# lionnus/I-ViT

Measured on AMD Instinct MI355X. Metric: images/sec DeiT-B INT8 @batch256, 1→8 MI355X; % INT8 MFMA peak, higher is better.
Workload: dtype int8; 1 GPU; DeiT-B INT8 integer-only forward, batch 256 per GPU, 224x224; global_batch=256, parallelism=dp1, launch=hip-graph replay, bitwidth=8, activation_ranges=power-of-two, operators=I-ViT (IVITIntLayerNorm, Shiftmax, ShiftGELU)

## Files before the change

### i-vit_amd/_lib.py

```python
from __future__ import annotations

import ctypes as C
import os
import subprocess

_HERE = os.path.dirname(os.path.abspath(__file__))
LIB_PATH = os.path.join(_HERE, "libivit_hip.so")
CSRC = os.path.join(_HERE, "csrc")

i64, i32, u32, f32, vp = C.c_int64, C.c_int32, C.c_uint32, C.c_float, C.c_void_p
ci = C.c_int

SIGNATURES = {
    "ivit_quantize_input_f32_i8": [vp, vp, i64, f32, vp],
    "ivit_quantize_patchify_f32_i8": [vp, vp, ci, ci, ci, ci, f32, vp],
    "ivit_gemm_i8_requant": [vp, i64, vp, i64, vp, vp, vp, vp, i64, ci, ci, ci, vp],
    "ivit_gemm_i8_requant_residual": [vp, i64, vp, i64, vp, vp, vp, vp, i64, u32, i32, u32, i32, vp, i64, ci, ci, ci, vp],
    "ivit_attention_fused_i8_ex": [vp, vp, ci, ci, ci, ci, u32, i32, f32, u32, i32, ci, vp],
    "ivit_layernorm_i8_ex": [vp, i64, ci, ci, vp, vp, vp, vp, vp, i64, ci, vp],
    "ivit_layernorm_i8_compat": [vp, i64, ci, ci, vp, vp, vp, vp, vp, vp, vp, i64, ci, vp],
    "ivit_attention_fused_i8_compat": [vp, vp, ci, ci, ci, ci, u32, i32, f32, u32, i32, vp, ci, vp],
    "ivit_attention_fused_i8_compat_band": [vp, vp, ci, ci, ci, ci, u32, i32, f32, u32, i32, vp, vp, ci, ci, vp],
    "ivit_attention_fused_i8_wide": [vp, vp, ci, ci, ci, ci, u32, i32, f32, u32, i32, vp, vp, ci, ci, ci, vp],
    "ivit_attention_fused_i8_long": [vp, vp, ci, ci, ci, ci, u32, i32, f32, u32, i32, vp, vp, ci, ci, vp],
# ... 60 lines not shown
    "ivit_ibert_gelu_build_lut": [f32, f32, f32, f32, f32, u32, i32, vp, vp],
    "ivit_ibert_softmax_build_table": [f32, f32, f32, f32, f32, f32, u32, i32, vp, vp],
    "ivit_attention_fused_i8_ibert": [vp, vp, ci, ci, ci, ci, u32, i32, u32, i32, vp, vp, ci, ci, vp],
    "ivit_attention_fused_i8_ibert_wide": [vp, vp, ci, ci, ci, ci, u32, i32, u32, i32, vp, vp, ci, ci, ci, vp],
    "ivit_attention_fused_i8_ibert_long": [vp, vp, ci, ci, ci, ci, u32, i32, u32, i32, vp, vp, ci, ci, vp],
    "ivit_ibert_layernorm_i8": [vp, i64, ci, ci, f32, vp, vp, f32, vp, vp, vp, i64, ci, vp],
    "ivit_ibert_layernorm_i16_i8": [vp, i64, ci, ci, f32, vp, vp, f32, vp, vp, vp, i64, vp],
    "ivit_ibert_layernorm_i16_i8_ex": [vp, i64, ci, ci, f32, vp, vp, f32, vp, vp, vp, i64, ci, vp],
    "ivit_ibert_gelu_f32_f32": [vp, i64, f32, f32, f32, f32, f32, vp, vp],
    "ivit_ibert_softmax_f32_f32": [vp, i64, ci, ci, f32, f32, f32, f32, f32, f32, u32, i32, ci, vp, i64, vp, vp],
    "ivit_ibert_layernorm_f32_f32": [vp, i64, ci, ci, vp, ci, vp, vp, f32, vp, i64, vp],
    "ivit_window_attention_i8": [vp, vp, i64, vp, vp, ci, ci, ci, ci, ci, ci, u32, i32, u32, i32, f32, u32, i32, vp],
    "ivit_window_attention_i8_compat": [vp, vp, i64, vp, vp, ci, ci, ci, ci, ci, ci, u32, i32, u32, i32, f32, u32, i32, vp, vp, vp],
    "ivit_window_attention_i8_band": [vp, vp, i64, vp, vp, ci, ci, ci, ci, ci, u32, i32, u32, i32, f32, u32, i32, vp, ci, ci, ci, ci, ci, ci, vp],
    "ivit_window_attention_i8_unwindow": [vp, vp, i64, vp, vp, ci, ci, ci, ci, ci, ci, u32, i32, u32, i32, f32, u32, i32, vp, vp,
                                          ci, ci, ci, ci, vp],
    "ivit_window_attention_i8_long": [vp, vp, i64, vp, vp, ci, ci, ci, ci, ci, ci, u32, i32, u32, i32, f32, u32, i32, vp, vp, vp, ci,
                                      ci, ci, ci, ci, ci, ci, vp],
    "ivit_eval_geometry": [ci, ci, ci, ci, vp],
    "ivit_resize_crop_workspace": [vp, ci, ci, vp, vp],
    "ivit_resize_crop_bicubic_u8": [vp, vp, vp, ci, ci, ci, ci, ci, vp, i64, vp, vp],
    "ivit_jpeg_probe": [vp, i64, vp],
    "ivit_jpeg_plan_image": [vp, i64, vp, i64, vp],
    "ivit_jpeg_workspace": [vp, i64, vp, vp, ci, vp, vp],
    "ivit_jpeg_decode_host": [vp, i64, vp, i64],
    "ivit_jpeg_decode_u8": [vp, vp, ci, i64, i64, i64, vp, i64, vp, vp, vp],
}


LAB_SIGNATURES = {
    "ivit_debug_force_small_gemm": [ci],
    "ivit_debug_set_gemm_flags": [ci],
    "ivit_debug_set_gemm_flags2": [ci],
    "ivit_debug_ln_wave_per_row": [ci],
    "ivit_debug_ln_ablate": [ci],
    "ivit_debug_ln_stream_cfg": [ci],
    "ivit_debug_ln_stamp_buffer": [vp],
    "ivit_gemm_i8_requant_gelu_ex": [vp, i64, vp, i64, vp, vp, vp, vp, vp, vp, i64, ci, ci, ci, ci, vp],
    "ivit_gemm_gelu_workspace_bytes": [ci, vp],
    "ivit_debug_set_stamp_buffer": [vp],
}
LAB_PATH = os.path.join(_HERE, "libivit_hip_lab.so")


class IvitError(RuntimeError):
    pass


def build(force: bool = False, verbose: bool = False) -> str:
    cmd = ["make", "-C", CSRC, "-j4"] + (["-B"] if force else []) + ([] if verbose else ["-s"])
    subprocess.check_call(cmd)
    return LIB_PATH


_lib = None
_lab = None
_use_lab = os.environ.get("IVIT_USE_LAB_LIBRARY") == "1"


def _load(path, signatures):
    if not os.path.exists(path):
        raise IvitError(f"{path} is missing: run `python -c 'import __graft_entry__ as g; g.build()'` "
                        "(there is no CPU / PyTorch fallback for the integer ViT path)")
    L = C.CDLL(path)
    L.ivit_version.restype = ci
    L.ivit_last_error_string.restype = C.c_char_p
# ... 57 lines not shown
```

### i-vit_amd/csrc/check_resources.py

```python
#!/usr/bin/env python3
import re
import sys

GUARDED = ("gemm_i8_wreg_kernel", "gemm_i8_pers_kernel", "gemm_i8_wp_kernel")
FIELDS = {"VGPRs": r"\bVGPRs: (\d+)", "AGPRs": r"AGPRs: (\d+)", "Scratch": r"ScratchSize \[bytes/lane\]: (\d+)",
          "Occupancy": r"Occupancy \[waves/SIMD\]: (\d+)", "VGPRSpill": r"VGPRs Spill: (\d+)", "SGPRSpill": r"SGPRs Spill: (\d+)",
          "LDS": r"LDS Size \[bytes/block\]: (\d+)"}


def parse(text):
    kernels, cur = {}, None
    for line in text.splitlines():
        m = re.search(r"Function Name: (\S+)", line)
        if m:
            cur = kernels.setdefault(m.group(1), {})
            continue
        if cur is None:
            continue
        for k, pat in FIELDS.items():
            m = re.search(pat, line)
            if m and k not in cur:
                cur[k] = int(m.group(1))
    return kernels


def occupancy_rules(path, what):
    kernels = parse(open(path, errors="replace").read())
    bad, seen = [], 0
    for name, r in sorted(kernels.items()):
        if what == "attention" and "attention_long_kernel" in name:
            m = re.search(r"attention_long_kernelILi(\d+)ELb([01])ELi(\d+)ELi(\d+)E", name)
            occ, need_no_scratch = int(m.group(4)) // 256, True
        elif what == "attention" and "attention_cls_kernel" in name:
            occ, need_no_scratch = 3, True
        elif what == "attention":
            m = re.search(r"attention_kernelILi(\d+)ELi(\d+)ELi(\d+)ELb([01])E", name)
            if not m:
# ... 62 lines not shown
```

### i-vit_amd/csrc/gemm.hip

```cpp
#include <type_traits>
#include "gemm_common.h"

namespace {

template <int EPI>
__global__ __launch_bounds__(NT) void gemm_i8_kernel(GemmArgs g)
{
    __shared__ __attribute__((aligned(16))) char smem[SMEM_BYTES + BN * 8];

    const int nblk = g.tiles_m * g.tiles_n;
    const int bid = blockIdx.x;
    const int q8 = nblk >> 3, r8 = nblk & 7, xcd = bid & 7;
    const int lid = (xcd < r8 ? xcd * (q8 + 1) : r8 * (q8 + 1) + (xcd - r8) * q8) + (bid >> 3);
    const int tm = lid / g.tiles_n, tn = lid - tm * g.tiles_n;
    const int m0 = tm * BM, n0 = tn * BN;

    const int tid = threadIdx.x;
    const int lane = tid & 63, wave = tid >> 6;
    const int wm = wave >> 1, wn = wave & 1;
    const int h = lane >> 5, l31 = lane & 31;
    if constexpr (EPI != EPI_I32 && EPI != EPI_RQ16 && EPI != EPI_RQ16_RES16) fill_rq_table(g, smem + SMEM_BYTES, n0, BN, tid);

    const int srow = tid >> 2, sc = tid & 3;
    const int8_t* ap[2];
// ... 887 lines not shown
                }
            }
            if (__builtin_amdgcn_ballot_w64(unc != 0) != 0) {
#pragma unroll
                for (int ii = 0; ii < 4; ++ii) {
                    const int c0 = 16 * min(i0 + ii, nsub - 1) + 4 * g4;
#pragma unroll
                    for (int r = 0; r < 4; ++r) {
                        const double tq = (double)acc[ii][r] * dyadic_mult(g.m[c0 + r], g.e[c0 + r]) + IVIT_MAGIC;
                        b[ii][r] = clamp_i32((int)(unsigned)__double_as_longlong(tq), -128, 127);
                    }
                }
            }
            unsigned D[4];
#pragma unroll
            for (int ii = 0; ii < 4; ++ii)
                D[ii] = __builtin_amdgcn_perm((unsigned)b[ii][1], (unsigned)b[ii][0], 0x0c0c0400u) |
                        __builtin_amdgcn_perm((unsigned)b[ii][3], (unsigned)b[ii][2], 0x04000c0cu);
            typedef unsigned v2u __attribute__((ext_vector_type(2)));
            const v2u ab = __builtin_amdgcn_permlane32_swap(D[0], D[2], false, false);
            const v2u cd = __builtin_amdgcn_permlane32_swap(D[1], D[3], false, false);
            const v2u ac = __builtin_amdgcn_permlane16_swap(ab.x, cd.x, false, false);
            const v2u bd = __builtin_amdgcn_permlane16_swap(ab.y, cd.y, false, false);
            const int ci = i0 + g4;
            if (ci < nsub && t < g.M) {
                const int4 v = make_int4((int)ac.x, (int)ac.y, (int)bd.x, (int)bd.y);
                if constexpr (EPI == EPI_QKV) *reinterpret_cast<int4*>(out + coff[4 * ci] + qrow_off) = v;
                else *reinterpret_cast<int4*>(out + (int64_t)t * g.ldo + 16 * ci) = v;
            }
        }
    }
}

#include "gemm_wp.h"

template <int EPI>
int launch_gemm(GemmArgs& g, const char* name, ivit_stream_t stream, int qkv_planes = 3)
{
    IVIT_REQUIRE(g.A && g.W && g.out, "%s: NULL operand", name);
    IVIT_REQUIRE(g.M > 0 && g.N > 0 && g.K > 0, "%s: empty problem M=%d N=%d K=%d", name, g.M, g.N, g.K);
    IVIT_REQUIRE(g.K % BK == 0, "%s: K=%d must be a multiple of %d", name, g.K, BK);
    IVIT_REQUIRE(g.lda >= g.K && g.ldw >= g.K && g.lda % 16 == 0 && g.ldw % 16 == 0,
                 "%s: lda=%lld ldw=%lld must be >= K and multiples of 16", name, (long long)g.lda, (long long)g.ldw);
    IVIT_REQUIRE(((uintptr_t)g.A % 16 == 0) && ((uintptr_t)g.W % 16 == 0) && ((uintptr_t)g.out % 16 == 0),
                 "%s: operands must be 16-byte aligned", name);
    if (EPI == EPI_I32 || EPI == EPI_RQ16 || EPI == EPI_RQ16_RES16) {
        IVIT_REQUIRE(g.N % 4 == 0 && g.ldo % 4 == 0 && g.ldo >= g.N, "%s: N=%d ldo=%lld must be multiples of 4", name,
                     g.N, (long long)g.ldo);
        if (EPI == EPI_RQ16 || EPI == EPI_RQ16_RES16)
            IVIT_REQUIRE(g.m && g.e && ((uintptr_t)g.m % 16 == 0) && ((uintptr_t)g.e % 16 == 0) && ((uintptr_t)g.out % 8 == 0),
                         "%s: requantiser tables missing or misaligned", name);
    } else {
        IVIT_REQUIRE(g.m && g.e, "%s: NULL requantiser table", name);
        IVIT_REQUIRE(((uintptr_t)g.bias % 16 == 0), "%s: bias must be 16-byte aligned", name);
        IVIT_REQUIRE(g.N % 16 == 0, "%s: N=%d must be a multiple of 16", name, g.N);
        IVIT_REQUIRE(((uintptr_t)g.m % 16 == 0) && ((uintptr_t)g.e % 16 == 0), "%s: m/e tables must be 16-byte aligned",
                     name);
    }
    if (EPI == EPI_RQ || EPI == EPI_RESID)
        IVIT_REQUIRE(g.ldo >= g.N && g.ldo % 16 == 0, "%s: ldo=%lld must be >= N and a multiple of 16", name,
                     (long long)g.ldo);
    if (EPI == EPI_RESID)
        IVIT_REQUIRE(g.res && g.ldr >= g.N && g.ldr % 16 == 0 && ((uintptr_t)g.res % 16 == 0),
                     "%s: residual operand missing or misaligned", name);
    if (EPI == EPI_RESID16 || EPI == EPI_RQ16_RES16)
        IVIT_REQUIRE(g.res && g.ldr >= g.N && g.ldr % 8 == 0 && ((uintptr_t)g.res % 16 == 0) && g.ldo >= g.N && g.ldo % 8 == 0,
                     "%s: 16-bit residual / output rows must be 16-byte aligned (ld multiples of 8 elements)", name);
    if (EPI == EPI_QKV) {
        IVIT_REQUIRE(g.tokens > 0 && g.heads > 0 && g.head_dim > 0 && g.head_dim % 16 == 0,
                     "%s: bad head geometry tokens=%d heads=%d head_dim=%d", name, g.tokens, g.heads, g.head_dim);
        IVIT_REQUIRE((int64_t)g.M * g.N < 2147483648ll, "%s: q/k/v output of %lld bytes exceeds the 2 GiB the 32-bit head-major offsets cover",
                     name, (long long)g.M * g.N);
        IVIT_REQUIRE(g.N == qkv_planes * g.heads * g.head_dim && g.M % g.tokens == 0,
                     "%s: N=%d != %d*heads*head_dim or M=%d %% tokens=%d != 0", name, g.N, qkv_planes, g.M, g.tokens);
    }
    g.flags = g_debug_flags & (31 | 128 | 256 | 512);
    g.flags2 = g_debug_flags2;
#if IVIT_LAB
    g.stamp = reinterpret_cast<unsigned long long*>(g_stamp_buf);
#endif
    const bool blocks = g.a_blocks || g.w_blocks;
    if constexpr (EPI == EPI_RQ || EPI == EPI_QKV) {
        if (!blocks && !g.w_frags && !g.out_blocks && !g.lut && !g.gelu_ws && g.M >= 8192 && g.K >= 32 && g.K <= SK_MAXK && g.K % 32 == 0 && g.N >= 16 &&
            g.N <= SK_MAXN && g.N % 16 == 0 && g.lda % 16 == 0 && g.ldw % 8 == 0 && ((uintptr_t)g.A % 16 == 0) && ((uintptr_t)g.W % 8 == 0) &&
            ((uintptr_t)g.out % 16 == 0) && (EPI == EPI_QKV || g.ldo % 16 == 0) && (EPI != EPI_QKV || g.head_dim % 16 == 0) && (int64_t)g.M * (EPI == EPI_QKV ? g.N : g.ldo) < 4294967296ll &&
            !g_force_small && !(IVIT_LAB && ((g_debug_flags2 & (1 << 20)) || (g_debug_flags & (31 | 128 | 256 | 512 | 1024))))) {
            const int nstrips = (g.M + 15) >> 4;
            const int grid = (nstrips + SK_WPB - 1) / SK_WPB < 512 ? (nstrips + SK_WPB - 1) / SK_WPB : 512;
            const bool any_k = IVIT_LAB && (g_debug_flags2 & (1 << 21));
            if (g.K == 128 && !any_k) hipLaunchKernelGGL((gemm_i8_skinny_kernel<EPI, 4>), dim3(grid), dim3(SK_NT), 0, ivit_stream(stream), g);
            else if (g.K == 64 && !any_k) hipLaunchKernelGGL((gemm_i8_skinny_kernel<EPI, 2>), dim3(grid), dim3(SK_NT), 0, ivit_stream(stream), g);
            else hipLaunchKernelGGL((gemm_i8_skinny_kernel<EPI, 0>), dim3(grid), dim3(SK_NT), 0, ivit_stream(stream), g);
            IVIT_CHECK_LAUNCH(name);
        }
    }
    if (blocks && !g.w_frags) {
        IVIT_REQUIRE(EPI != EPI_I32 && EPI != EPI_RQ16 && g.M >= 2048 && g.N >= BCH && !g_force_small,
                     "%s: block-layout operands need the persistent kernel (M >= 2048, N >= 128, requantising epilogue)", name);
        IVIT_REQUIRE(!g.a_blocks || g.lda == g.K, "%s: a block-layout A operand is dense (lda == K)", name);
        IVIT_REQUIRE(!g.w_blocks || g.ldw == g.K, "%s: a block-layout W operand is dense (ldw == K)", name);
    }
    if (g.w_frags) IVIT_REQUIRE(!g.a_blocks || g.lda == g.K, "%s: a block-layout A operand is dense (lda == K)", name);
    IVIT_REQUIRE(!g.lut || (g.w_frags && EPI == EPI_RQ), "%s: the output map needs the fragment-packed weight form (IVIT_W_FRAGS)", name);
    if (g.w_frags) {
        IVIT_REQUIRE(EPI != EPI_I32 && EPI != EPI_RQ16 && g.M >= 2048 && g.N >= 128 && g.N % 64 == 0 && (g.K / BK) % 3 == 0 && !g.w_blocks && !g_force_small,
                     "%s: the fragment-packed weight needs M >= 2048, N >= 128, N %% 64 == 0, K %% 192 == 0 and a requantising epilogue", name);
        if constexpr (EPI != EPI_I32 && EPI != EPI_RQ16) {
            g.tiles_m = (g.M + WR_TOK - 1) / WR_TOK;
            g.tiles_n = (g.N + WR_CH - 1) / WR_CH;
            g.narrow = 0;
            if constexpr (EPI == EPI_RQ || EPI == EPI_RESID || EPI == EPI_QKV) {
                if (IVIT_LAB && g.w_frags == 2 && !g.lut && !g.gelu_ws && (g_debug_flags2 & 8192) && !(g_debug_flags2 & (256 | 512))) {
                    g.narrow = 1;
                    g.tiles_n = (g.N + WR_CH / 2 - 1) / (WR_CH / 2);
                }
            }
            const int ntiles = g.tiles_m * g.tiles_n;
            if constexpr (IVIT_LAB != 0 && (EPI == EPI_RQ || EPI == EPI_QKV)) {
                if (g.w_frags == 2 && !g.lut && !g.gelu_ws && !g.narrow && (g.K / BK) >= 12 && (g_debug_flags2 & 32768) && !(g_debug_flags2 & (256 | 512)) &&
                    !(g_debug_flags & 127)) {
                    IVIT_REQUIRE(((int64_t)g.M + 16) * (EPI == EPI_QKV ? g.N : g.ldo) < 4294967296ll,
                                 "%s: IVIT_W_FRAGS16 addresses its output with 32-bit offsets: operand of 4 GiB or more", name);
                    g.split_from = ntiles;
                    if constexpr (EPI == EPI_QKV) {
                        IVIT_REQUIRE((int64_t)g.M * g.tokens < 4294967296ll, "%s: M * tokens must stay below 2^32", name);
// ... 385 lines not shown
```

### i-vit_amd/csrc/gemm_common.h

```cpp
#pragma once
#include <type_traits>

#include "common.h"

#if IVIT_LAB
extern int g_kernel_choice;
extern bool g_force_small;
extern void* g_stamp_buf;
extern int g_debug_flags;
extern int g_debug_flags2;
#else
constexpr int g_kernel_choice = 0;
constexpr bool g_force_small = false;
constexpr int g_debug_flags = 0;
constexpr int g_debug_flags2 = 0;
#endif
#ifndef IVIT_STORE_POLICY
#define IVIT_STORE_POLICY 0
#endif

namespace {

constexpr int BM = 128;
constexpr int BN = 128;
constexpr int BK = 64;
constexpr int NT = 256;
constexpr int STAGE_BYTES = (BM + BN) * BK;
constexpr int W_OFF = BM * BK;
constexpr int SMEM_BYTES = 2 * STAGE_BYTES;

enum { EPI_RQ = 0, EPI_RESID = 1, EPI_QKV = 2, EPI_I32 = 3, EPI_RESID16 = 4, EPI_RQ16 = 5, EPI_RQ16_RES16 = 6 };


struct GemmArgs {
    const int8_t* A;
    int64_t lda;
    const int8_t* W;
    int64_t ldw;
    const int32_t* bias;
    const uint32_t* m;
    const int32_t* e;
    void* out;
    int64_t ldo;
// ... 934 lines not shown
```

### i-vit_amd/csrc/gemm_lab.hip

```cpp
#include "gemm_common.h"

int g_kernel_choice = 0;
bool g_force_small = false;
void* g_stamp_buf = nullptr;
int g_debug_flags = 0;
int g_debug_flags2 = 0;

namespace {

template <int EPI, int ABL>
__global__ __launch_bounds__(BIG_NT, 2) void gemm_i8_big_kernel(GemmArgs g)
{
    __shared__ __attribute__((aligned(16))) char smem[BIG_SMEM + BCH * 8];
    unsigned long long t_start = 0, t_loop = 0, t_epi = 0, r_start = 0;
    if constexpr (ABL & 512) {
        t_start = __builtin_amdgcn_s_memtime();
        r_start = __builtin_amdgcn_s_memrealtime();
    }

    const int nblk = g.tiles_m * g.tiles_n;
    const int bid = blockIdx.x;
    const int q8 = nblk >> 3, r8 = nblk & 7, xcd = bid & 7;
    const int lid = (xcd < r8 ? xcd * (q8 + 1) : r8 * (q8 + 1) + (xcd - r8) * q8) + (bid >> 3);
    const int tm = lid / g.tiles_n, tn = lid - tm * g.tiles_n;
    const int m0 = tm * BTOK, n0 = tn * BCH;

    const int tid = threadIdx.x;
    const int lane = tid & 63, wave = __builtin_amdgcn_readfirstlane(tid >> 6);
    const int wc = wave >> 1, wt = wave & 1;
    const int h = lane >> 5, l31 = lane & 31;

    const int8_t* asrc[4];
    const int8_t* wsrc[2];
    const int lrow = lane >> 2, lslot = lane & 3;
#pragma unroll
    for (int i = 0; i < 4; ++i) {
        int row = 16 * (wave + 4 * i) + lrow;
        int c = lslot ^ ((row >> 2) & 3);
        asrc[i] = g.A + (int64_t)min(m0 + row, g.M - 1) * g.lda + 16 * c;
// ... 189 lines not shown

int ivit_gemm_lab_launch(int epi, void* gemm_args, const char* name, ivit_stream_t stream, int* rc)
{
    GemmArgs& g = *static_cast<GemmArgs*>(gemm_args);
    int handled = 0;
    switch (epi) {
        case EPI_RQ: *rc = launch_lab<EPI_RQ>(g, name, stream, &handled); break;
        case EPI_RESID: *rc = launch_lab<EPI_RESID>(g, name, stream, &handled); break;
        case EPI_QKV: *rc = launch_lab<EPI_QKV>(g, name, stream, &handled); break;
        default: break;
    }
    return handled;
}

IVIT_EXPORT int ivit_debug_force_small_gemm(int on)
{
    g_force_small = (on == 1);
    g_kernel_choice = (on == 2);
    return IVIT_OK;
}

IVIT_EXPORT int ivit_debug_set_gemm_flags(int flags)
{
    g_debug_flags = flags;
    return IVIT_OK;
}

IVIT_EXPORT int ivit_debug_set_gemm_flags2(int flags)
{
    g_debug_flags2 = flags;
    return IVIT_OK;
}

IVIT_EXPORT int ivit_debug_set_stamp_buffer(void* buf)
{
    g_stamp_buf = buf;
    return IVIT_OK;
}
```

### i-vit_amd/csrc/rowops.hip

```cpp
#include <limits.h>

#include "common.h"
#include "rowsum.h"

#if IVIT_LAB
int g_ln_wave_per_row = 0;
int g_ln_ablate = 0;
int g_ln_stream_cfg = 0;
unsigned long long* g_ln_stamps = nullptr;
#else
constexpr int g_ln_wave_per_row = 0;
constexpr int g_ln_ablate = 0;
constexpr int g_ln_stream_cfg = 0;
#endif

namespace {

typedef float v2f __attribute__((ext_vector_type(2)));

constexpr int NT = 256;
constexpr int WPB = NT / 64;

IVIT_DEV int sx8(int v, int byte) { return (int)(int8_t)(v >> (8 * byte)); }

// ... 1023 lines not shown
    if (total < 2147483648ll) {
        const unsigned w4 = (unsigned)(hw >> 2), tot = (unsigned)total;
        for (unsigned q = blockIdx.x * NT + threadIdx.x; q < tot; q += gridDim.x * NT) {
            const unsigned r = q / w4, x4 = q - r * w4;
            const unsigned r2 = r / (unsigned)hw, y = r - r2 * (unsigned)hw;
            const unsigned b = r2 / (unsigned)chans, c = r2 - b * (unsigned)chans;
            const float4 v = *reinterpret_cast<const float4*>(img + (size_t)r * hw + 4 * x4);
            const unsigned px = x4 / (unsigned)pw4, kw = (x4 - px * pw4) * 4;
            const unsigned py = y / (unsigned)patch, kh = y - py * patch;
            const int64_t row = ((int64_t)b * g + py) * g + px;
            const unsigned col = (c * patch + kh) * patch + kw;
            *reinterpret_cast<int*>(A + row * lda + col) = pack4(quant_sym_i8(v.x, inv_scale), quant_sym_i8(v.y, inv_scale),
                                                                 quant_sym_i8(v.z, inv_scale), quant_sym_i8(v.w, inv_scale));
        }
        return;
    }
    for (int64_t q = (int64_t)blockIdx.x * NT + threadIdx.x; q < total; q += (int64_t)gridDim.x * NT) {
        int x4 = (int)(q % (hw >> 2));
        int64_t r = q / (hw >> 2);
        int y = (int)(r % hw);
        r /= hw;
        int c = (int)(r % chans);
        int b = (int)(r / chans);
        float4 v = *reinterpret_cast<const float4*>(img + (((int64_t)b * chans + c) * hw + y) * hw + 4 * x4);
        int px = x4 / pw4, kw = (x4 - px * pw4) * 4;
        int py = y / patch, kh = y - py * patch;
        int64_t row = ((int64_t)b * g + py) * g + px;
        int col = (c * patch + kh) * patch + kw;
        *reinterpret_cast<int*>(A + row * lda + col) = pack4(quant_sym_i8(v.x, inv_scale), quant_sym_i8(v.y, inv_scale),
                                                             quant_sym_i8(v.z, inv_scale), quant_sym_i8(v.w, inv_scale));
    }
}

__global__ __launch_bounds__(NT) void patchify_u8_kernel(const uint8_t* img, int8_t* A, int64_t lda, int batch, int chans, int hw,
                                                         int patch, const int8_t* lut)
{
    __shared__ int8_t s_lut[4 * 256];
    for (int i = threadIdx.x; i < chans * 256; i += NT) s_lut[i] = lut[i];
    __syncthreads();
    const int g = hw / patch;
    const int pw4 = patch >> 2;
    const int64_t total = (int64_t)batch * chans * hw * (hw >> 2);
    for (int64_t q = (int64_t)blockIdx.x * NT + threadIdx.x; q < total; q += (int64_t)gridDim.x * NT) {
        int x4 = (int)(q % (hw >> 2));
        int64_t r = q / (hw >> 2);
        int y = (int)(r % hw);
        r /= hw;
        int c = (int)(r % chans);
        int b = (int)(r / chans);
        const unsigned v = *reinterpret_cast<const unsigned*>(img + (((int64_t)b * chans + c) * hw + y) * hw + 4 * x4);
        const int8_t* t = s_lut + 256 * c;
        int px = x4 / pw4, kw = (x4 - px * pw4) * 4;
        int py = y / patch, kh = y - py * patch;
        int64_t row = ((int64_t)b * g + py) * g + px;
        int col = (c * patch + kh) * patch + kw;
        *reinterpret_cast<int*>(A + row * lda + col) = pack4(t[v & 255], t[(v >> 8) & 255], t[(v >> 16) & 255], t[v >> 24]);
    }
}

__global__ __launch_bounds__(NT) void embed_kernel(const int8_t* patch, const int16_t* pos_add, const int8_t* cls_row,
                                                   double Mq, int8_t* out, int batch, int tokens, int C)
{
    const int cd = C >> 2;
    const int64_t total = (int64_t)batch * tokens * cd;
    for (int64_t q = (int64_t)blockIdx.x * NT + threadIdx.x; q < total; q += (int64_t)gridDim.x * NT) {
        int d = (int)(q % cd);
        int64_t r = q / cd;
        int tok = (int)(r % tokens);
        int b = (int)(r / tokens);
        int res;
        if (tok == 0) {
            res = *reinterpret_cast<const int*>(cls_row + 4 * d);
        } else {
            int w = *reinterpret_cast<const int*>(patch + ((int64_t)b * (tokens - 1) + tok - 1) * C + 4 * d);
            const int16_t* pa = pos_add + (int64_t)tok * C + 4 * d;
            int o[4];
#pragma unroll
            for (int c = 0; c < 4; ++c) o[c] = clamp_i32(requant_exact(sx8(w, c), Mq) + (int)pa[c], -128, 127);
            res = pack4(o[0], o[1], o[2], o[3]);
        }
        *reinterpret_cast<int*>(out + ((int64_t)b * tokens + tok) * C + 4 * d) = res;
    }
}

__global__ __launch_bounds__(NT) void embed16_kernel(const int16_t* patch, const int32_t* pos_add, const int16_t* cls_row,
                                                     double Mq, int16_t* out, int batch, int tokens, int C)
{
    const int cd = C >> 2;
    const int64_t total = (int64_t)batch * tokens * cd;
    for (int64_t q = (int64_t)blockIdx.x * NT + threadIdx.x; q < total; q += (int64_t)gridDim.x * NT) {
        const int d = (int)(q % cd);
        const int64_t r = q / cd;
        const int tok = (int)(r % tokens);
        const int b = (int)(r / tokens);
        int2 res;
        if (tok == 0) {
            res = *reinterpret_cast<const int2*>(cls_row + 4 * d);
        } else {
            const int2 w = *reinterpret_cast<const int2*>(patch + ((int64_t)b * (tokens - 1) + tok - 1) * C + 4 * d);
            const int4 pa = *reinterpret_cast<const int4*>(pos_add + (int64_t)tok * C + 4 * d);
            const int k[4] = {(int)(int16_t)w.x, w.x >> 16, (int)(int16_t)w.y, w.y >> 16};
            const int p4[4] = {pa.x, pa.y, pa.z, pa.w};
            int o[4];
#pragma unroll
            for (int c = 0; c < 4; ++c) o[c] = clamp_i32(requant_exact(k[c], Mq) + p4[c], -32768, 32767);
            res.x = (o[0] & 0xffff) | (o[1] << 16);
            res.y = (o[2] & 0xffff) | (o[3] << 16);
        }
        *reinterpret_cast<int2*>(out + ((int64_t)b * tokens + tok) * C + 4 * d) = res;
    }
}

__global__ __launch_bounds__(NT) void head_argmax_kernel(const int32_t* acc, const float* s_acc, int batch, int N,
                                                         float* logits, int32_t* top1)
// ... 641 lines not shown
    hipLaunchKernelGGL(minmax_kernel, dim3(ew_grid(n) < 2048 ? ew_grid(n) : 2048), dim3(NT), 0, st, x, n, keys);
    hipLaunchKernelGGL(minmax_finish_kernel, dim3(1), dim3(1), 0, st, keys);
    IVIT_CHECK_LAUNCH("ivit_minmax_f32");
}

IVIT_EXPORT int ivit_quantize_input_f32_i8(const float* x, int8_t* out, int64_t n, float inv_scale,
                                           ivit_stream_t stream)
{
    IVIT_REQUIRE(x && out && n > 0, "ivit_quantize_input_f32_i8: bad operand");
    IVIT_REQUIRE(((uintptr_t)x % 16 == 0) && ((uintptr_t)out % 4 == 0), "ivit_quantize_input_f32_i8: misaligned");
    hipLaunchKernelGGL(quantize_kernel, dim3(ew_grid(n / 4 + 1)), dim3(NT), 0, ivit_stream(stream), x, out, n,
                       inv_scale);
    IVIT_CHECK_LAUNCH("ivit_quantize_input_f32_i8");
}

IVIT_EXPORT int ivit_quantize_input_f32_i32(const float* x, int32_t* out, int64_t n, float inv_scale, int bits,
                                            ivit_stream_t stream)
{
    IVIT_REQUIRE(x && out && n > 0 && bits >= 2 && bits <= 32, "ivit_quantize_input_f32_i32: bad operand");
    const float lo = -__builtin_ldexpf(1.0f, bits - 1), hi = __builtin_ldexpf(1.0f, bits - 1) - 1.0f;
    hipLaunchKernelGGL(quantize_i32_kernel, dim3(ew_grid(n)), dim3(NT), 0, ivit_stream(stream), x, out, n, inv_scale, lo, hi);
    IVIT_CHECK_LAUNCH("ivit_quantize_input_f32_i32");
}

static int launch_patchify(const char* who, const float* img, int8_t* A, int64_t lda, int batch, int chans, int hw, int patch,
                           float inv_scale, ivit_stream_t stream)
{
    IVIT_REQUIRE(img && A && batch > 0 && chans > 0, "%s: bad operand", who);
    IVIT_REQUIRE(patch > 0 && patch % 4 == 0 && hw % patch == 0, "%s: hw=%d patch=%d", who, hw, patch);
    IVIT_REQUIRE(lda >= (int64_t)chans * patch * patch && lda % 4 == 0, "%s: lda=%lld too small or not a multiple of 4", who,
                 (long long)lda);
    IVIT_REQUIRE(((uintptr_t)img % 16 == 0) && ((uintptr_t)A % 4 == 0), "%s: misaligned", who);
    const int64_t total = (int64_t)batch * chans * hw * (hw / 4);
    hipLaunchKernelGGL(patchify_kernel, dim3(ew_grid(total)), dim3(NT), 0, ivit_stream(stream), img, A, lda, batch, chans,
                       hw, patch, inv_scale);
    IVIT_CHECK_LAUNCH(who);
}

IVIT_EXPORT int ivit_quantize_patchify_f32_i8(const float* img, int8_t* A, int batch, int chans, int hw, int patch,
                                              float inv_scale, ivit_stream_t stream)
{
    return launch_patchify("ivit_quantize_patchify_f32_i8", img, A, (int64_t)chans * patch * patch, batch, chans, hw, patch,
                           inv_scale, stream);
}

IVIT_EXPORT int ivit_quantize_patchify_u8_i8(const uint8_t* img, int8_t* A, int64_t lda, int batch, int chans, int hw, int patch,
                                             const int8_t* lut, ivit_stream_t stream)
{
    IVIT_REQUIRE(img && A && lut && batch > 0 && chans > 0 && chans <= 4 && hw > 0 && patch > 0 && hw % patch == 0 && patch % 4 == 0,
                 "ivit_quantize_patchify_u8_i8: bad shape (up to 4 channels, hw %% patch == 0, patch %% 4 == 0)");
    IVIT_REQUIRE(lda >= (int64_t)chans * patch * patch && lda % 4 == 0 && ((uintptr_t)img % 4 == 0) && ((uintptr_t)A % 4 == 0),
                 "ivit_quantize_patchify_u8_i8: lda too small or misaligned operand");
    const int64_t total = (int64_t)batch * chans * hw * (hw / 4);
    hipLaunchKernelGGL(patchify_u8_kernel, dim3(ew_grid(total)), dim3(NT), 0, ivit_stream(stream), img, A, lda, batch, chans, hw,
                       patch, lut);
    IVIT_CHECK_LAUNCH("ivit_quantize_patchify_u8_i8");
}

IVIT_EXPORT int ivit_quantize_patchify_ld_f32_i8(const float* img, int8_t* A, int64_t lda, int batch, int chans, int hw,
                                                 int patch, float inv_scale, ivit_stream_t stream)
{
    return launch_patchify("ivit_quantize_patchify_ld_f32_i8", img, A, lda, batch, chans, hw, patch, inv_scale, stream);
}

IVIT_EXPORT int ivit_embed_assemble_i8(const int8_t* patch, const int16_t* pos_add, const int8_t* cls_row, uint32_t m,
                                       int32_t e, int8_t* out, int batch, int tokens, int C, ivit_stream_t stream)
{
    IVIT_REQUIRE(patch && pos_add && cls_row && out, "ivit_embed_assemble_i8: NULL operand");
    IVIT_REQUIRE(batch > 0 && tokens > 1 && C > 0 && C % 4 == 0, "ivit_embed_assemble_i8: bad shape");
    IVIT_REQUIRE(((uintptr_t)patch % 4 == 0) && ((uintptr_t)out % 4 == 0) && ((uintptr_t)cls_row % 4 == 0) &&
                     ((uintptr_t)pos_add % 8 == 0),
                 "ivit_embed_assemble_i8: misaligned");
    const double Mq = ivit_dyadic_to_double(m, e);
    IVIT_REQUIRE(Mq < 1048576.0, "ivit_embed_assemble_i8: requant multiplier too large");
    const int64_t total = (int64_t)batch * tokens * (C / 4);
    hipLaunchKernelGGL(embed_kernel, dim3(ew_grid(total)), dim3(NT), 0, ivit_stream(stream), patch, pos_add, cls_row,
                       Mq, out, batch, tokens, C);
    IVIT_CHECK_LAUNCH("ivit_embed_assemble_i8");
}

IVIT_EXPORT int ivit_embed_assemble_i16(const int16_t* patch, const int32_t* pos_add, const int16_t* cls_row, uint32_t m,
                                        int32_t e, int16_t* out, int batch, int tokens, int C, ivit_stream_t stream)
{
    IVIT_REQUIRE(patch && pos_add && cls_row && out, "ivit_embed_assemble_i16: NULL operand");
    IVIT_REQUIRE(batch > 0 && tokens > 1 && C > 0 && C % 4 == 0, "ivit_embed_assemble_i16: bad shape");
    IVIT_REQUIRE(((uintptr_t)patch % 8 == 0) && ((uintptr_t)out % 8 == 0) && ((uintptr_t)cls_row % 8 == 0) &&
                     ((uintptr_t)pos_add % 16 == 0),
                 "ivit_embed_assemble_i16: misaligned");
    const double Mq = ivit_dyadic_to_double(m, e);
    IVIT_REQUIRE(Mq < 32768.0, "ivit_embed_assemble_i16: requant multiplier too large");
    const int64_t total = (int64_t)batch * tokens * (C / 4);
    hipLaunchKernelGGL(embed16_kernel, dim3(ew_grid(total)), dim3(NT), 0, ivit_stream(stream), patch, pos_add, cls_row,
                       Mq, out, batch, tokens, C);
    IVIT_CHECK_LAUNCH("ivit_embed_assemble_i16");
}

IVIT_EXPORT int ivit_head_argmax(const int32_t* acc, const float* s_acc, int batch, int N, float* logits_f32,
                                 int32_t* top1, ivit_stream_t stream)
{
    IVIT_REQUIRE(acc && s_acc && top1 && batch > 0 && N > 0, "ivit_head_argmax: bad operand");
    hipLaunchKernelGGL(head_argmax_kernel, dim3(grid_for_rows(batch)), dim3(NT), 0, ivit_stream(stream), acc, s_acc,
                       batch, N, logits_f32, top1);
    IVIT_CHECK_LAUNCH("ivit_head_argmax");
}

namespace {
template <bool F32>
void launch_head_topk(int k, const int32_t* acc, const float* s_acc, const float* logits_in, int batch, int ld, int N,
// ... 126 lines not shown
```

### include/ivit_hip_debug.h

```cpp
#ifndef IVIT_HIP_DEBUG_H
#define IVIT_HIP_DEBUG_H

#ifdef __cplusplus
extern "C" {
#endif

int ivit_debug_force_small_gemm(int on);
int ivit_debug_set_gemm_flags(int flags);
int ivit_debug_set_gemm_flags2(int flags);
int ivit_debug_set_stamp_buffer(void* buf);

int ivit_debug_ln_wave_per_row(int on);

int ivit_debug_ln_stream_cfg(int cfg);
int ivit_debug_ln_stamp_buffer(void* buf);

int ivit_debug_ln_ablate(int bits);

int ivit_gemm_gelu_workspace_bytes(int M, int64_t* bytes);
int ivit_gemm_i8_requant_gelu_ex(const int8_t* A, int64_t lda, const int8_t* W, int64_t ldw, const int32_t* bias,
                                 const uint32_t* m, const int32_t* e, const int8_t* gelu_lut, void* workspace,
                                 int8_t* out, int64_t ldo, int M, int N, int K, int layouts, ivit_stream_t stream);

#ifdef __cplusplus
}
#endif
#endif
```

Before: 42160 images/s.

## Add split-K small-M GEMM kernel and vectorized patchify/embed streaming kernels

Adds a small-M int8 GEMM kernel that tiles output as 64x32 and splits the K loop across four waves. Each wave keeps a register-prefetched pipeline of MFMA operands, then partial sums are reduced through LDS before a requant, residual or int32 epilogue. It is selected for small M/N tile counts, such as the classifier head, where the existing kernels leave most of the GPU idle. Patchify and embed-assemble also get 16-byte-per-thread streaming kernels when alignment allows. These add code paths and a debug launch counter, with some risk in the new dispatch conditions and edge handling.

Result: no change. 42560 images/s, median of 6 (+0.9%).

```diff
diff --git a/i-vit_amd/_lib.py b/i-vit_amd/_lib.py
--- a/i-vit_amd/_lib.py
+++ b/i-vit_amd/_lib.py
@@ -116,6 +116,7 @@
     "ivit_debug_force_small_gemm": [ci],
     "ivit_debug_set_gemm_flags": [ci],
     "ivit_debug_set_gemm_flags2": [ci],
+    "ivit_debug_small_m_gemm_launches": [vp],
     "ivit_debug_ln_wave_per_row": [ci],
     "ivit_debug_ln_ablate": [ci],
     "ivit_debug_ln_stream_cfg": [ci],
diff --git a/i-vit_amd/csrc/check_resources.py b/i-vit_amd/csrc/check_resources.py
--- a/i-vit_amd/csrc/check_resources.py
+++ b/i-vit_amd/csrc/check_resources.py
@@ -2,7 +2,8 @@
 import re
 import sys
 
-GUARDED = ("gemm_i8_wreg_kernel", "gemm_i8_pers_kernel", "gemm_i8_wp_kernel")
+GUARDED = ("gemm_i8_wreg_kernel", "gemm_i8_pers_kernel", "gemm_i8_wp_kernel",
+           "gemm_i8_smallm_kernel")
 FIELDS = {"VGPRs": r"\bVGPRs: (\d+)", "AGPRs": r"AGPRs: (\d+)", "Scratch": r"ScratchSize \[bytes/lane\]: (\d+)",
           "Occupancy": r"Occupancy \[waves/SIMD\]: (\d+)", "VGPRSpill": r"VGPRs Spill: (\d+)", "SGPRSpill": r"SGPRs Spill: (\d+)",
           "LDS": r"LDS Size \[bytes/block\]: (\d+)"}
diff --git a/i-vit_amd/csrc/gemm.hip b/i-vit_amd/csrc/gemm.hip
--- a/i-vit_amd/csrc/gemm.hip
+++ b/i-vit_amd/csrc/gemm.hip
@@ -943,6 +943,151 @@
     }
 }
 
+constexpr int SM_ROWS = 64, SM_CH = 32, SM_NT = 256, SM_DEPTH = 4;
+constexpr int SM_MAX_M = 1024, SM_MAX_ITEMS = 384;
+constexpr int SM_RS = SM_CH + 4;
+constexpr int SM_SMEM = 4 * SM_ROWS * SM_RS * 4;
+
+template <int EPI>
+__global__ __launch_bounds__(SM_NT) void gemm_i8_smallm_kernel(GemmArgs g)
+{
+    static_assert(EPI == EPI_RQ || EPI == EPI_RESID || EPI == EPI_I32, "small-M form: plain int8, residual and raw int32 epilogues");
+    __shared__ __attribute__((aligned(16))) int part[4 * SM_ROWS * SM_RS];
+    const int tid = threadIdx.x, lane = tid & 63, wave = tid >> 6;
+    const int g4 = lane >> 4, l15 = lane & 15;
+    const int tn = blockIdx.x % g.tiles_n, tm = blockIdx.x / g.tiles_n;
+    const int m0 = tm * SM_ROWS, n0 = tn * SM_CH;
+
+    const int orow = m0 + (tid >> 2), och = n0 + 8 * (tid & 3);
+    const bool o_ok = orow < g.M && och < g.N;
+    const bool o_ok2 = o_ok && och + 4 < g.N;
+    int bv[8] = {0, 0, 0, 0, 0, 0, 0, 0};
+    uint32_t mv[8];
+    int32_t ev[8];
+    int2 rv = make_int2(0, 0);
+    if (o_ok) {
+        if (g.bias) {
+            const int4 b0 = *reinterpret_cast<const int4*>(g.bias + och);
+            bv[0] = b0.x; bv[1] = b0.y; bv[2] = b0.z; bv[3] = b0.w;
+            if (EPI != EPI_I32 || o_ok2) {
+                const int4 b1 = *reinterpret_cast<const int4*>(g.bias + och + 4);
+                bv[4] = b1.x; bv[5] = b1.y; bv[6] = b1.z; bv[7] = b1.w;
+            }
+        }
+        if constexpr (EPI != EPI_I32) {
+            const uint4 ma = *reinterpret_cast<const uint4*>(g.m + och), mb = *reinterpret_cast<const uint4*>(g.m + och + 4);
+            const int4 ea = *reinterpret_cast<const int4*>(g.e + och), eb = *reinterpret_cast<const int4*>(g.e + och + 4);
+            mv[0] = ma.x; mv[1] = ma.y; mv[2] = ma.z; mv[3] = ma.w; mv[4] = mb.x; mv[5] = mb.y; mv[6] = mb.z; mv[7] = mb.w;
+            ev[0] = ea.x; ev[1] = ea.y; ev[2] = ea.z; ev[3] = ea.w; ev[4] = eb.x; ev[5] = eb.y; ev[6] = eb.z; ev[7] = eb.w;
+        }
+        if constexpr (EPI == EPI_RESID) rv = *reinterpret_cast<const int2*>(g.res + (int64_t)orow * g.ldr + och);
+    }
+
+    const int nk = g.K / BK, kq = nk >> 2, kr = nk & 3;
+    const int ns = kq + (wave < kr ? 1 : 0), k0 = wave * kq + min(wave, kr);
+    v4i acc[2][4];
+#pragma unroll
+    for (int i = 0; i < 2; ++i)
+#pragma unroll
+        for (int j = 0; j < 4; ++j) acc[i][j] = v4i{0, 0, 0, 0};
+    if (ns > 0) {
+        const int8_t* ap[4];
+        const int8_t* wp[2];
+        int astep = BK;
+#pragma unroll
+        for (int j = 0; j < 4; ++j) {
+            const int64_t r = min(m0 + 16 * j + l15, g.M - 1);
+            if (g.a_blocks) {
+                const int64_t pr = r * (g.lda / g.K);
+                const int rl = (int)(pr & 15);
+                ap[j] = g.A + ((pr >> 4) * nk + k0) * 1024 + (((rl << 2) + (g4 ^ ((rl >> 2) & 3))) << 4);
+            } else {
+                ap[j] = g.A + r * g.lda + (int64_t)k0 * BK + 16 * g4;
+            }
+        }
+        if (g.a_blocks) astep = 1024;
+#pragma unroll
+        for (int i = 0; i < 2; ++i)
+            wp[i] = g.W + (int64_t)min(n0 + 16 * i + l15, g.N - 1) * g.ldw + (int64_t)k0 * BK + 16 * g4;
+        v4i fa[SM_DEPTH][4], fw[SM_DEPTH][2];
+#pragma unroll
+        for (int d = 0; d < SM_DEPTH; ++d) {
+            const int s = min(d, ns - 1);
+#pragma unroll
+            for (int i = 0; i < 2; ++i) fw[d][i] = *reinterpret_cast<const v4i*>(wp[i] + (int64_t)s * BK);
+#pragma unroll
+            for (int j = 0; j < 4; ++j) fa[d][j] = *reinterpret_cast<const v4i*>(ap[j] + (int64_t)s * astep);
+        }
+        auto step = [&](int d) {
+#pragma unroll
+            for (int i = 0; i < 2; ++i)
+#pragma unroll
+                for (int j = 0; j < 4; ++j)
+                    acc[i][j] = __builtin_amdgcn_mfma_i32_16x16x64_i8(fw[d][i], fa[d][j], acc[i][j], 0, 0, 0);
+        };
+        auto refill = [&](int d, int s) {
+#pragma unroll
+            for (int i = 0; i < 2; ++i) fw[d][i] = *reinterpret_cast<const v4i*>(wp[i] + (int64_t)s * BK);
+#pragma unroll
+            for (int j = 0; j < 4; ++j) fa[d][j] = *reinterpret_cast<const v4i*>(ap[j] + (int64_t)s * astep);
+        };
+        int s0 = 0;
+        for (; s0 + 2 * SM_DEPTH <= ns; s0 += SM_DEPTH) {
+#pragma unroll
+            for (int d = 0; d < SM_DEPTH; ++d) {
+                step(d);
+                refill(d, s0 + d + SM_DEPTH);
+            }
+        }
+#pragma unroll
+        for (int d = 0; d < SM_DEPTH; ++d) {
+            if (s0 + d < ns) {
+                step(d);
+                if (s0 + d + SM_DEPTH < ns) refill(d, s0 + d + SM_DEPTH);
+            }
+        }
+#pragma unroll
+        for (int d = 0; d < SM_DEPTH; ++d)
+            if (s0 + SM_DEPTH + d < ns) step(d);
+        int* const pw = part + wave * (SM_ROWS * SM_RS);
+#pragma unroll
+        for (int i = 0; i < 2; ++i)
+#pragma unroll
+            for (int j = 0; j < 4; ++j) *reinterpret_cast<v4i*>(pw + (16 * j + l15) * SM_RS + 16 * i + 4 * g4) = acc[i][j];
+    }
+    __syncthreads();
+    if (!o_ok) return;
+    const int nparts = nk < 4 ? nk : 4;
+    int sum[8];
+#pragma unroll
+    for (int c = 0; c < 8; ++c) sum[c] = bv[c];
+    for (int w = 0; w < nparts; ++w) {
+        const int* p = part + w * (SM_ROWS * SM_RS) + (tid >> 2) * SM_RS + 8 * (tid & 3);
+        const v4i p0 = *reinterpret_cast<const v4i*>(p), p1 = *reinterpret_cast<const v4i*>(p + 4);
+        sum[0] += p0.x; sum[1] += p0.y; sum[2] += p0.z; sum[3] += p0.w;
+        sum[4] += p1.x; sum[5] += p1.y; sum[6] += p1.z; sum[7] += p1.w;
+    }
+    if constexpr (EPI == EPI_I32) {
+        int32_t* out = reinterpret_cast<int32_t*>(g.out) + (int64_t)orow * g.ldo + och;
+        *reinterpret_cast<int4*>(out) = make_int4(sum[0], sum[1], sum[2], sum[3]);
+        if (o_ok2) *reinterpret_cast<int4*>(out + 4) = make_int4(sum[4], sum[5], sum[6], sum[7]);
+    } else {
+        int o[8];
+#pragma unroll
+        for (int c = 0; c < 8; ++c) {
+            const double p = (double)sum[c] * dyadic_mult(mv[c], ev[c]);
+            const double t = p + IVIT_MAGIC;
+            o[c] = clamp_i32((int)(unsigned)__double_as_longlong(t), -128, 127);
+            if constexpr (EPI == EPI_RESID) {
+                const int xr = (int)(int8_t)((c < 4 ? rv.x : rv.y) >> (8 * (c & 3)));
+                o[c] = clamp_i32(requant_exact(o[c], g.M_main) + requant_exact(xr, g.M_res), -128, 127);
+            }
+        }
+        *reinterpret_cast<int2*>(reinterpret_cast<int8_t*>(g.out) + (int64_t)orow * g.ldo + och) =
+            make_int2(pack4_i8(o[0], o[1], o[2], o[3]), pack4_i8(o[4], o[5], o[6], o[7]));
+    }
+}
+
 #include "gemm_wp.h"
 
 template <int EPI>
@@ -1002,6 +1147,21 @@
             if (g.K == 128 && !any_k) hipLaunchKernelGGL((gemm_i8_skinny_kernel<EPI, 4>), dim3(grid), dim3(SK_NT), 0, ivit_stream(stream), g);
             else if (g.K == 64 && !any_k) hipLaunchKernelGGL((gemm_i8_skinny_kernel<EPI, 2>), dim3(grid), dim3(SK_NT), 0, ivit_stream(stream), g);
             else hipLaunchKernelGGL((gemm_i8_skinny_kernel<EPI, 0>), dim3(grid), dim3(SK_NT), 0, ivit_stream(stream), g);
+            IVIT_CHECK_LAUNCH(name);
+        }
+    }
+    if constexpr (EPI == EPI_RQ || EPI == EPI_RESID || EPI == EPI_I32) {
+        const bool lab_other = IVIT_LAB && (g_force_small || (g_debug_flags2 & (1 << 22)) || (g_debug_flags & (31 | 128 | 256 | 512 | 1024)));
+        const bool any_m = IVIT_LAB && (g_debug_flags2 & (1 << 23));
+        const int64_t items = (int64_t)((g.M + SM_ROWS - 1) / SM_ROWS) * ((g.N + SM_CH - 1) / SM_CH);
+        if (((g.M <= SM_MAX_M && items <= SM_MAX_ITEMS) || any_m || (g.a_blocks && g.lda != g.K && g.M < 2048)) && !lab_other && !g.w_blocks && !g.w_frags && !g.lut && !g.out_blocks && !g.gelu_ws &&
+            (!g.a_blocks || (g.lda != g.K && g.lda % g.K == 0)) && ((uintptr_t)g.bias % 16 == 0) && items < 2147483648ll) {
+            g.tiles_m = (g.M + SM_ROWS - 1) / SM_ROWS;
+            g.tiles_n = (g.N + SM_CH - 1) / SM_CH;
+#if IVIT_LAB
+            ++g_small_m_launches;
+#endif
+            hipLaunchKernelGGL(gemm_i8_smallm_kernel<EPI>, dim3(g.tiles_m * g.tiles_n), dim3(SM_NT), 0, ivit_stream(stream), g);
             IVIT_CHECK_LAUNCH(name);
         }
     }
diff --git a/i-vit_amd/csrc/gemm_common.h b/i-vit_amd/csrc/gemm_common.h
--- a/i-vit_amd/csrc/gemm_common.h
+++ b/i-vit_amd/csrc/gemm_common.h
@@ -9,6 +9,7 @@
 extern void* g_stamp_buf;
 extern int g_debug_flags;
 extern int g_debug_flags2;
+extern long long g_small_m_launches;
 #else
 constexpr int g_kernel_choice = 0;
 constexpr bool g_force_small = false;
diff --git a/i-vit_amd/csrc/gemm_lab.hip b/i-vit_amd/csrc/gemm_lab.hip
--- a/i-vit_amd/csrc/gemm_lab.hip
+++ b/i-vit_amd/csrc/gemm_lab.hip
@@ -5,6 +5,7 @@
 void* g_stamp_buf = nullptr;
 int g_debug_flags = 0;
 int g_debug_flags2 = 0;
+long long g_small_m_launches = 0;
 
 namespace {
 
@@ -260,6 +261,13 @@
     return IVIT_OK;
 }
 
+IVIT_EXPORT int ivit_debug_small_m_gemm_launches(int64_t* count)
+{
+    IVIT_REQUIRE(count, "ivit_debug_small_m_gemm_launches: NULL result");
+    *count = g_small_m_launches;
+    return IVIT_OK;
+}
+
 IVIT_EXPORT int ivit_debug_set_stamp_buffer(void* buf)
 {
     g_stamp_buf = buf;
diff --git a/i-vit_amd/csrc/rowops.hip b/i-vit_amd/csrc/rowops.hip
--- a/i-vit_amd/csrc/rowops.hip
+++ b/i-vit_amd/csrc/rowops.hip
@@ -1079,6 +1079,27 @@
     }
 }
 
+__global__ __launch_bounds__(NT) void patchify_stream_kernel(const float* img, int8_t* A, int64_t lda, unsigned nrows, unsigned chans,
+                                                             unsigned hw, unsigned patch, float inv_scale)
+{
+    const unsigned g = hw / patch, p16 = patch >> 4, cpr = chans * patch * p16, tot = nrows * cpr;
+    for (unsigned u = blockIdx.x * NT + threadIdx.x; u < tot; u += gridDim.x * NT) {
+        const unsigned row = u / cpr, cc = u - row * cpr;
+        const unsigned t = cc / p16, kw16 = cc - t * p16;
+        const unsigned c = t / patch, kh = t - c * patch;
+        const unsigned bp = row / g, px = row - bp * g;
+        const unsigned b = bp / g, py = bp - b * g;
+        const float4* src = reinterpret_cast<const float4*>(img + ((size_t)(b * chans + c) * hw + (py * patch + kh)) * hw + px * patch + 16 * kw16);
+        const float4 v0 = src[0], v1 = src[1], v2 = src[2], v3 = src[3];
+        int4 o;
+        o.x = pack4(quant_sym_i8(v0.x, inv_scale), quant_sym_i8(v0.y, inv_scale), quant_sym_i8(v0.z, inv_scale), quant_sym_i8(v0.w, inv_scale));
+        o.y = pack4(quant_sym_i8(v1.x, inv_scale), quant_sym_i8(v1.y, inv_scale), quant_sym_i8(v1.z, inv_scale), quant_sym_i8(v1.w, inv_scale));
+        o.z = pack4(quant_sym_i8(v2.x, inv_scale), quant_sym_i8(v2.y, inv_scale), quant_sym_i8(v2.z, inv_scale), quant_sym_i8(v2.w, inv_scale));
+        o.w = pack4(quant_sym_i8(v3.x, inv_scale), quant_sym_i8(v3.y, inv_scale), quant_sym_i8(v3.z, inv_scale), quant_sym_i8(v3.w, inv_scale));
+        *reinterpret_cast<int4*>(A + (int64_t)row * lda + 16 * cc) = o;
+    }
+}
+
 __global__ __launch_bounds__(NT) void patchify_u8_kernel(const uint8_t* img, int8_t* A, int64_t lda, int batch, int chans, int hw,
                                                          int patch, const int8_t* lut)
 {
@@ -1127,6 +1148,40 @@
             res = pack4(o[0], o[1], o[2], o[3]);
         }
         *reinterpret_cast<int*>(out + ((int64_t)b * tokens + tok) * C + 4 * d) = res;
+    }
+}
+
+__global__ __launch_bounds__(NT) void embed_stream_kernel(const int8_t* patch, const int16_t* pos_add, const int8_t* cls_row,
+                                                          double Mq, int8_t* out, unsigned rows, unsigned tokens, unsigned cpr)
+{
+    const unsigned tot = rows * cpr;
+    for (unsigned q = blockIdx.x * NT + threadIdx.x; q < tot; q += gridDim.x * NT) {
+        const unsigned r = q / cpr, d = q - r * cpr;
+        const unsigned b = r / tokens, tok = r - b * tokens;
+        int4 res;
+        if (tok == 0) {
+            res = *reinterpret_cast<const int4*>(cls_row + 16 * d);
+        } else {
+            const int4 w4 = *reinterpret_cast<const int4*>(patch + ((size_t)(r - b - 1) * cpr + d) * 16);
+            const int4* pa = reinterpret_cast<const int4*>(pos_add + ((size_t)tok * cpr + d) * 16);
+            const int4 p0 = pa[0], p1 = pa[1];
+            const int w[4] = {w4.x, w4.y, w4.z, w4.w};
+            const int pp[8] = {p0.x, p0.y, p0.z, p0.w, p1.x, p1.y, p1.z, p1.w};
+            int ow[4];
+#pragma unroll
+            for (int k = 0; k < 4; ++k) {
+                int o[4];
+#pragma unroll
+                for (int c = 0; c < 4; ++c) {
+                    const int pw = pp[2 * k + (c >> 1)];
+                    const int pav = (c & 1) ? (pw >> 16) : (int)(int16_t)pw;
+                    o[c] = clamp_i32(requant_exact(sx8(w[k], c), Mq) + pav, -128, 127);
+                }
+                ow[k] = pack4(o[0], o[1], o[2], o[3]);
+            }
+            res = make_int4(ow[0], ow[1], ow[2], ow[3]);
+        }
+        *reinterpret_cast<int4*>(out + (size_t)q * 16) = res;
     }
 }
 
@@ -1834,6 +1889,12 @@
                  (long long)lda);
     IVIT_REQUIRE(((uintptr_t)img % 16 == 0) && ((uintptr_t)A % 4 == 0), "%s: misaligned", who);
     const int64_t total = (int64_t)batch * chans * hw * (hw / 4);
+    if (patch % 16 == 0 && total / 4 < 2147483648ll && lda % 16 == 0 && ((uintptr_t)A % 16 == 0)) {
+        const int g = hw / patch;
+        hipLaunchKernelGGL(patchify_stream_kernel, dim3((unsigned)((total / 4 + NT - 1) / NT)), dim3(NT), 0, ivit_stream(stream), img, A, lda,
+                           (unsigned)(batch * g * g), (unsigned)chans, (unsigned)hw, (unsigned)patch, inv_scale);
+        IVIT_CHECK_LAUNCH(who);
+    }
     hipLaunchKernelGGL(patchify_kernel, dim3(ew_grid(total)), dim3(NT), 0, ivit_stream(stream), img, A, lda, batch, chans,
                        hw, patch, inv_scale);
     IVIT_CHECK_LAUNCH(who);
@@ -1876,6 +1937,12 @@
     const double Mq = ivit_dyadic_to_double(m, e);
     IVIT_REQUIRE(Mq < 1048576.0, "ivit_embed_assemble_i8: requant multiplier too large");
     const int64_t total = (int64_t)batch * tokens * (C / 4);
+    if (C % 16 == 0 && total / 4 < 2147483648ll && ((uintptr_t)patch % 16 == 0) && ((uintptr_t)out % 16 == 0) && ((uintptr_t)cls_row % 16 == 0) &&
+        ((uintptr_t)pos_add % 16 == 0)) {
+        hipLaunchKernelGGL(embed_stream_kernel, dim3((unsigned)((total / 4 + NT - 1) / NT)), dim3(NT), 0, ivit_stream(stream), patch, pos_add,
+                           cls_row, Mq, out, (unsigned)(batch * tokens), (unsigned)tokens, (unsigned)(C / 16));
+        IVIT_CHECK_LAUNCH("ivit_embed_assemble_i8");
+    }
     hipLaunchKernelGGL(embed_kernel, dim3(ew_grid(total)), dim3(NT), 0, ivit_stream(stream), patch, pos_add, cls_row,
                        Mq, out, batch, tokens, C);
     IVIT_CHECK_LAUNCH("ivit_embed_assemble_i8");
diff --git a/include/ivit_hip_debug.h b/include/ivit_hip_debug.h
--- a/include/ivit_hip_debug.h
+++ b/include/ivit_hip_debug.h
@@ -8,6 +8,7 @@
 int ivit_debug_force_small_gemm(int on);
 int ivit_debug_set_gemm_flags(int flags);
 int ivit_debug_set_gemm_flags2(int flags);
+int ivit_debug_small_m_gemm_launches(int64_t* count);
 int ivit_debug_set_stamp_buffer(void* buf);
 
 int ivit_debug_ln_wave_per_row(int on);
```
